# fgvieira/ngsF-HMM

Measured on AMD Instinct MI355X. Metric: site-ind updates/sec (EM iterations x individuals x sites / s), 1M sites x 1k ind, higher is better.
Workload: dtype f64

## Files before the change

### ngsf-hmm_amd/csrc/kernels_fast_estmaf.hip

```cpp
#include "fast_dev.hpp"

#include <mutex>

namespace capi {
void set_error(const char* fmt, ...);
}

namespace nghmm {

namespace {



__device__ double2 estmaf_term_logspace(const double* g, double freq, double F) {
  double h[3];
  h[0] = (1 - freq) * (1 - freq) + (1 - freq) * freq * F;
  h[1] = 2 * (1 - freq) * freq - 2 * (1 - freq) * freq * F;
  h[2] = freq * freq + (1 - freq) * freq * F;
  double pp[3];
  for (int k = 0; k < 3; ++k) {
    double l = log(h[k]);
    if (l == -__builtin_huge_val()) l = -kINF;
    h[k] = l;
  }
// ... 39 lines not shown
  {
    const uint64_t b = ngh_bits(v);
    const int lo = __builtin_amdgcn_update_dpp(0, (int)(uint32_t)b, 0x143, 0xc, 0xf, false);
    const int hi = __builtin_amdgcn_update_dpp(0, (int)(uint32_t)(b >> 32), 0x143, 0xc, 0xf, false);
    v += ngh_from_bits(((uint64_t)(uint32_t)hi << 32) | (uint32_t)lo);
  }
  return v;
}

__device__ __forceinline__ double wave_sum_uniform(double v) {
  v += dpp_move<0xB1>(v);
  v += dpp_move<0x4E>(v);
  v += dpp_move<0x141>(v);
  v += dpp_move<0x140>(v);
  return ((lane_value(v, 0) + lane_value(v, 16)) + lane_value(v, 32)) + lane_value(v, 48);
}

__device__ __forceinline__ double wave_sum_pair(double pn, double pd) {
  const uint64_t bn = ngh_bits(pn), bd = ngh_bits(pd);
  const auto lo = __builtin_amdgcn_permlane32_swap((unsigned)bn, (unsigned)bd, false, false);
  const auto hi = __builtin_amdgcn_permlane32_swap((unsigned)(bn >> 32), (unsigned)(bd >> 32),
                                                   false, false);
  double v = ngh_from_bits(((uint64_t)hi[0] << 32) | lo[0]) +
             ngh_from_bits(((uint64_t)hi[1] << 32) | lo[1]);
  v += dpp_move<0xB1>(v);
  v += dpp_move<0x4E>(v);
  v += dpp_move<0x141>(v);
  v += dpp_move<0x140>(v);
  {
    const uint64_t b = ngh_bits(v);
    const int l = __builtin_amdgcn_update_dpp(0, (int)(uint32_t)b, 0x142, 0xa, 0xf, false);
    const int h = __builtin_amdgcn_update_dpp(0, (int)(uint32_t)(b >> 32), 0x142, 0xa, 0xf, false);
    v += ngh_from_bits(((uint64_t)(uint32_t)h << 32) | (uint32_t)l);
  }
  return v;
}

constexpr int EN = 12;
constexpr int EST_SCALARS = 8;
constexpr int EST_FIELDS = EST_SCALARS + 2 * EN;
enum : uint8_t { EST_DONE = 0, EST_INTERP = 1, EST_EXACT = 2 };
constexpr int EST_K0 = 2;
constexpr int EST_MIN_GAIN = 24;
constexpr double EST_DMAX = 0.85;
constexpr double EST_BACK = 0.1;
constexpr double EST_MULT = 32.0;
constexpr double EST_FIT = 0.72;
constexpr int EST_KMAX = 32;
constexpr double EST_TOL = 1e-11;
constexpr double EST_GUARD = 1e-9;
__constant__ double kChebC[EN] = {0.9914448613738104, 0.9238795325112867, 0.7933533402912352, 0.6087614290087207, 0.38268343236508984, 0.1305261922200517, -0.1305261922200516, -0.3826834323650895, -0.6087614290087207, -0.793353340291235, -0.9238795325112867, -0.9914448613738104};
__constant__ double kChebW[EN] = {0.13052619222005157, -0.3826834323650898, 0.6087614290087207, -0.7933533402912352, 0.9238795325112867, -0.9914448613738104, 0.9914448613738104, -0.9238795325112868, 0.7933533402912352, -0.6087614290087209, 0.3826834323650899, -0.130526192220052};

constexpr int ESTMAF_MAXW = 16;

__device__ __forceinline__ bool in_tile_rows(uint64_t site, uint64_t tile_T, uint64_t row0,
                                             uint64_t row1) {
  if (tile_T == 0) return true;
  const uint64_t j = site / tile_T, t = site - j * tile_T;
  const uint64_t row = (j >> 6) * tile_T + t;
  return row >= row0 && row < row1;
}
__host__ __device__ constexpr int estmaf_full_slots(int NI, int BLOCK) {
  return BLOCK == 64 ? (NI == 16 ? 12 : NI == 12 ? 8 : NI == 8 ? 4 : NI == 4 ? 2 : NI == 2 ? 1 : 0)
                     : (NI == 16 ? 8 : 0);
}

template <int NI, int BLOCK, bool TILE>
__device__ __forceinline__ void estmaf_site(
    const GlView& gl, const double* __restrict__ marg_blocks, uint64_t S_own, uint64_t I_tot,
    uint64_t I_blk, double* __restrict__ freq_out, uint8_t* __restrict__ redo,
    uint8_t* __restrict__ status, double* __restrict__ state, uint64_t state_stride, int fresh,
    int n_exact, int allow_build, uint64_t site, const double* __restrict__ tile_col,
    uint32_t* __restrict__ cnt, double (&xch)[2][ESTMAF_MAXW][2],
    double2 (&nodebuf)[(BLOCK == 64 && NI >= 8) ? EN : 1][(BLOCK == 64 && NI >= 8) ? 65 : 1],
    double2 (&xnode)[(BLOCK == 64 && NI >= 8) ? 1 : EN][(BLOCK == 64 && NI >= 8) ? 1 : BLOCK / 64],
    double2* park = nullptr) {
  constexpr int W = BLOCK / 64;
  constexpr bool PARK = (W == 1 && NI >= 8);
  const int lane = threadIdx.x & 63;
  const int wv = threadIdx.x >> 6;
  const uint32_t tix = threadIdx.x;
  constexpr uint64_t stride = BLOCK;
  const uint64_t cell_s = site * I_tot;

  double tF_lane_out;
  double sA[NI], sb[NI], sC[NI], u0[NI], nC[NI], fc[NI];
  {
    constexpr int NB = NI < 8 ? NI : (NI % 8 ? NI / 2 : 8);
    static_assert(NI % NB == 0, "whole batches");
    const bool one_block = (I_blk == I_tot);
    const uint32_t ib = (uint32_t)I_blk;
    double tF_acc = 0;
#pragma unroll
    for (int k0 = 0; k0 < NI; k0 += NB) {
      double r0[NB], r1[NB], r2[NB], rF[NB];
      uint64_t ic[NB];
#pragma unroll
      for (int j = 0; j < NB; ++j) {
        const uint64_t i = (uint64_t)tix + stride * (k0 + j);
        ic[j] = (k0 + j < estmaf_full_slots(NI, BLOCK) || i < I_tot) ? i : I_tot - 1;
        gl_fetch(gl, cell_s + ic[j], r0[j], r1[j], r2[j]);
      }
      if constexpr (TILE) {
#pragma unroll
        for (int j = 0; j < NB; ++j)
          rF[j] = tile_col[k0 + j < estmaf_full_slots(NI, BLOCK)
// ... 47 lines not shown
    num = state[0 * state_stride + site];
    den = state[1 * state_stride + site];
    pnum = state[2 * state_stride + site];
    pden = state[3 * state_stride + site];
    iters = (int)state[4 * state_stride + site];
  }
  bool built = !allow_build;
  int n_before = n_exact;
  bool check = false, interp_ok = false;
  double mid = 0, half = 0, my_gn = 0, my_gd = 0, rprev = 0;
  auto lane_sums = [&](double r, double& pn, double& pd) {
    pn = 0;
    pd = 0;
    if constexpr (NI >= 4) {
#pragma unroll
      for (int k0 = 0; k0 + 4 <= NI; k0 += 4) {
        double sm[4];
#pragma unroll
        for (int j = 0; j < 4; ++j) sm[j] = fma(r, fma(r, sC[k0 + j], sb[k0 + j]), sA[k0 + j]);
        const double p01 = sm[0] * sm[1], p23 = sm[2] * sm[3];
        const double R = rcp_nr(p01 * p23);
        const double r01 = R * p23, r23 = R * p01;
        const double inv0 = r01 * sm[1], inv1 = r01 * sm[0];
        const double inv2 = r23 * sm[3], inv3 = r23 * sm[2];
        pn = fma(fma(nC[k0], r, u0[k0]), inv0, pn);
        pd = fma(fc[k0], inv0, pd);
        pn = fma(fma(nC[k0 + 1], r, u0[k0 + 1]), inv1, pn);
        pd = fma(fc[k0 + 1], inv1, pd);
        pn = fma(fma(nC[k0 + 2], r, u0[k0 + 2]), inv2, pn);
        pd = fma(fc[k0 + 2], inv2, pd);
        pn = fma(fma(nC[k0 + 3], r, u0[k0 + 3]), inv3, pn);
        pd = fma(fc[k0 + 3], inv3, pd);
      }
      if constexpr (NI % 4 == 2) {
        constexpr int k0 = NI - 2;
        const double s0 = fma(r, fma(r, sC[k0], sb[k0]), sA[k0]);
        const double s1 = fma(r, fma(r, sC[k0 + 1], sb[k0 + 1]), sA[k0 + 1]);
        const double R = rcp_nr(s0 * s1);
        const double inv0 = R * s1, inv1 = R * s0;
        pn = fma(fma(nC[k0], r, u0[k0]), inv0, pn);
        pd = fma(fc[k0], inv0, pd);
        pn = fma(fma(nC[k0 + 1], r, u0[k0 + 1]), inv1, pn);
        pd = fma(fc[k0 + 1], inv1, pd);
      }
    } else {
#pragma unroll
      for (int k = 0; k < NI; ++k) {
        const double inv = rcp_nr(fma(r, fma(r, sC[k], sb[k]), sA[k]));
        pn = fma(fma(nC[k], r, u0[k]), inv, pn);
        pd = fma(fc[k], inv, pd);
      }
    }
  };
  for (;;) {
    const double r = pnum * rcp_nr2(pden - pnum);
    double pn, pd;
    lane_sums(r, pn, pd);
    const double v = wave_sum_pair(pn, pd);
    double sn = lane_value(v, 31), sd = lane_value(v, 63);
    if constexpr (W > 1) {
      if (lane == 0) {
        xch[buf][wv][0] = sn;
        xch[buf][wv][1] = sd;
      }
      __syncthreads();
      sn = xch[buf][0][0];
      sd = xch[buf][0][1];
#pragma unroll
      for (int w = 1; w < W; ++w) {
        sn += xch[buf][w][0];
        sd += xch[buf][w][1];
      }
      buf ^= 1;
    }
    if (check) {
      const int nj = lane < EN ? lane : 0;
      const double t = (r - mid) / (r + mid) - half * kChebC[nj];
      const double q = (lane < EN) ? kChebW[nj] / t : 0.0;
      const double Sq = wave_sum_uniform(q);
      const double bn = wave_sum_uniform(q * my_gn) / Sq, bd = wave_sum_uniform(q * my_gd) / Sq;
      interp_ok = fabs(bn - sn) <= EST_TOL * fabs(sn) && fabs(bd - sd) <= EST_TOL * fabs(sd);
      check = false;
      if (!interp_ok && tix == 0) atomicAdd(cnt + EST_CNT_CHECK_FAILED, 1u);
    }
    num = fma(r, sn, num);
    den = fma(r, sd, den + tF_sum);
    const double lhs = fabs(fma(pnum, den, -(num * pden))), thr = kEPS * (den * pden);
    const bool again = (lhs > thr) && (iters++ < 100);
    rprev = r;
    pnum = num;
    pden = den;
    if (!again) break;
    if (interp_ok) {
      if (wv == 0) {
        if (lane < EN) {
          state[(EST_SCALARS + lane) * state_stride + site] = my_gn;
          state[(EST_SCALARS + EN + lane) * state_stride + site] = my_gd;
        }
        if (lane == 0) {
          state[0 * state_stride + site] = num;
          state[1 * state_stride + site] = den;
          state[2 * state_stride + site] = pnum;
          state[3 * state_stride + site] = pden;
          state[4 * state_stride + site] = (double)iters;
          state[5 * state_stride + site] = mid;
          state[6 * state_stride + site] = half;
          state[7 * state_stride + site] = tF_sum;
          status[site] = EST_INTERP;
        }
      }
      return;
    }
    if (!built && --n_before <= 0) {
      const double m_est = (double)iters * (sqrt(lhs / thr) - 1.0);
      const double rn = pnum * rcp_nr2(pden - pnum);
      const double step = fabs(rn - rprev);
      const double reach = (rn >= rprev) ? EST_DMAX * rn : EST_DMAX / (1 + EST_DMAX) * rn;
      const bool fits = (double)iters * step <= EST_FIT * reach;
      if (!fits && iters < EST_KMAX && m_est >= EST_MIN_GAIN) {
        n_before = 1;
      } else {
        built = true;
      }
      if (built && m_est >= EST_MIN_GAIN && 100 - iters >= EST_MIN_GAIN) {
        const double g = fmin(EST_DMAX, fmax(EST_MULT * step / rn, 1e-3));
        double lo, hi;
        if (rn >= rprev) {
          lo = rn * (1 - EST_BACK * g);
          hi = rn * (1 + g);
        } else {
          lo = rn / (1 + g);
          hi = rn * (1 + EST_BACK * g);
        }
        mid = sqrt(lo * hi);
        half = (hi - mid) / (hi + mid);
        if (half > 0 && lo > 0 && hi < 1e300) {
          if constexpr (PARK) {
            const double tnl = half * kChebC[lane < EN ? lane : 0];
            const double r_nodes = mid * (1 + tnl) * rcp_nr2(1 - tnl);
#pragma unroll 1
            for (int nd = 0; nd < EN; ++nd) {
              double pn, pd;
              lane_sums(lane_value(r_nodes, nd), pn, pd);
              nodebuf[nd][lane] = double2{pn, pd};
            }
            __syncthreads();
            const int j = lane & 15, q4 = lane >> 4;
            double an = 0, ad = 0;
            if (j < EN) {
#pragma unroll
              for (int l = 0; l < 16; ++l) {
                const double2 t2 = nodebuf[j][q4 * 16 + l];
                an += t2.x;
                ad += t2.y;
              }
            }
            an += __shfl_xor(an, 16);
            ad += __shfl_xor(ad, 16);
            an += __shfl_xor(an, 32);
            ad += __shfl_xor(ad, 32);
            my_gn = an;
            my_gd = ad;
            check = true;
          } else {
            const double tnl = half * kChebC[lane < EN ? lane : 0];
            const double r_nodes = mid * (1 + tnl) * rcp_nr2(1 - tnl);
            double an = 0, ad = 0;
            if constexpr (W > 1) {
#pragma unroll 1
              for (int nd = 0; nd < EN; ++nd) {
                double pn, pd;
                lane_sums(lane_value(r_nodes, nd), pn, pd);
                park[nd * BLOCK + (int)tix] = double2{pn, pd};
              }
              __syncthreads();
              for (int nd = wv; nd < EN; nd += W) {
                double sn = 0, sd = 0;
#pragma unroll
                for (int w = 0; w < W; ++w) {
                  const double2 t2 = park[nd * BLOCK + w * 64 + lane];
                  sn += t2.x;
                  sd += t2.y;
                }
                const double v = wave_sum_pair(sn, sd);
                const double tn = lane_value(v, 31), td = lane_value(v, 63);
                if (lane == 0) xnode[nd][0] = double2{tn, td};
              }
              __syncthreads();
              if (lane < EN) {
                an = xnode[lane][0].x;
                ad = xnode[lane][0].y;
              }
              __syncthreads();
            } else {
#pragma unroll 1
              for (int nd = 0; nd < EN; ++nd) {
                double pn, pd;
                lane_sums(lane_value(r_nodes, nd), pn, pd);
                const double v = wave_sum_pair(pn, pd);
                const double sn = lane_value(v, 31), sd = lane_value(v, 63);
                if (lane == nd) {
                  an = sn;
                  ad = sd;
                }
              }
            }
            my_gn = an;
            my_gd = ad;
            check = true;
          }
        }
      }
    }
  }
  if (tix == 0) {
    const double freq = num / den;
    const bool ok = freq >= 0 && freq < 1;
    freq_out[site] = freq;
    redo[site] = ok ? 0 : 1;
    status[site] = EST_DONE;
  }
}

__device__ __forceinline__ const double* estmaf_tile_col(const double* marg_blocks, uint64_t site,
                                                         uint64_t tile_T, uint64_t I_tot) {
  const uint64_t j = site / tile_T, t = site - j * tile_T;
  return marg_blocks + post_lane_off((j >> 6) * tile_T + t, j & 63, I_tot);
}

#define ESTMAF_SHARED(NI, BLOCK)                                                              \
  constexpr bool PARK_ = ((BLOCK) == 64 && (NI) >= 8);                                         \
  __shared__ double xch[2][ESTMAF_MAXW][2];                       \
  __shared__ double2 nodebuf[PARK_ ? EN : 1][PARK_ ? 65 : 1];                                  \
  __shared__ double2 xnode[PARK_ ? 1 : EN][PARK_ ? 1 : (BLOCK) / 64]

template <int NI, int BLOCK, bool TILE>
__global__ void __launch_bounds__(BLOCK) __attribute__((amdgpu_waves_per_eu(2)))
k_fast_estmaf(const GlView gl, const double* __restrict__ marg_blocks,
              uint64_t S_own, uint64_t I_tot, uint64_t I_blk, uint64_t tile_T,
              double* __restrict__ freq_out, uint8_t* __restrict__ redo,
              uint8_t* __restrict__ status, double* __restrict__ state, uint64_t state_stride,
              int n_exact, int allow_build, uint64_t blk0, uint32_t* __restrict__ cnt) {
  ESTMAF_SHARED(NI, BLOCK);
  uint64_t site;
  const double* tile_col = nullptr;
  if constexpr (TILE) {
    const uint64_t b = blockIdx.x + blk0, x = b & 7, k = b >> 3;
    const uint64_t q = ((k >> 3) << 6) + (x << 3) + (k & 7);
    const uint64_t tile_row = q >> 6, l = q & 63;
    const uint64_t c = tile_row / tile_T, t = tile_row - c * tile_T;
    site = (c * 64 + l) * tile_T + t;
    if (site >= S_own) return;
    tile_col = marg_blocks + post_lane_off(tile_row, l, I_tot);
  } else {
    site = blockIdx.x;
  }
  extern __shared__ double2 park_mem[];
  estmaf_site<NI, BLOCK, TILE>(gl, marg_blocks, S_own, I_tot, I_blk, freq_out, redo, status, state,
                               state_stride, 1, n_exact, allow_build, site, tile_col, cnt, xch, nodebuf,
                               xnode, park_mem);
}

template <int NI, int BLOCK, bool TILE>
__global__ void __launch_bounds__(BLOCK) __attribute__((amdgpu_waves_per_eu(2)))
k_fast_estmaf_resume(const GlView gl, const double* __restrict__ marg_blocks,
                     uint64_t S_own, uint64_t I_tot, uint64_t I_blk, uint64_t tile_T,
                     double* __restrict__ freq_out, uint8_t* __restrict__ redo,
                     uint8_t* __restrict__ status, double* __restrict__ state,
                     uint64_t state_stride, int n_exact, int allow_build, uint64_t row0,
                     uint64_t row1, uint32_t* __restrict__ cnt, int cnt_slot) {
  ESTMAF_SHARED(NI, BLOCK);
  extern __shared__ double2 park_mem[];
  const int lane = threadIdx.x & 63;
  for (uint64_t base = (uint64_t)blockIdx.x * 64; base < S_own; base += (uint64_t)gridDim.x * 64) {
    const uint64_t s = base + lane;
    const bool need = s < S_own && in_tile_rows(s, TILE ? tile_T : 0, row0, row1) &&
                      status[s] == EST_EXACT;
    uint64_t mask = __ballot(need);
    if (mask && threadIdx.x == 0) atomicAdd(cnt + cnt_slot, (uint32_t)__popcll(mask));
    if constexpr (BLOCK > 64) __syncthreads();
    while (mask) {
      const uint64_t site = base + (uint64_t)__builtin_ctzll(mask);
      mask &= mask - 1;
      const double* tile_col = TILE ? estmaf_tile_col(marg_blocks, site, tile_T, I_tot) : nullptr;
      estmaf_site<NI, BLOCK, TILE>(gl, marg_blocks, S_own, I_tot, I_blk, freq_out, redo, status,
                                   state, state_stride, 0, n_exact, allow_build, site, tile_col, cnt,
                                   xch, nodebuf, xnode, park_mem);
      if constexpr (BLOCK > 64) __syncthreads();
    }
  }
}

__device__ __forceinline__ double row_sum(double v) {
  v = __dadd_rn(v, dpp_move<0xB1>(v));
  v = __dadd_rn(v, dpp_move<0x4E>(v));
  v = __dadd_rn(v, dpp_move<0x141>(v));
  v = __dadd_rn(v, dpp_move<0x140>(v));
  return v;
}

template <int NI, bool TILE>
__device__ __forceinline__ void estmaf_rows_sites(
    const GlView& gl, const double* __restrict__ marg_blocks, uint64_t S_own, uint64_t I_tot,
    uint64_t I_blk, double* __restrict__ freq_out, uint8_t* __restrict__ redo,
    uint8_t* __restrict__ status, double* __restrict__ state, uint64_t state_stride, int fresh,
    int n_exact, int allow_build, uint64_t site, const double* __restrict__ tile_col, bool done,
    uint32_t* __restrict__ cnt) {
  static_assert(EN <= 16, "a row's lanes hold the interval's node sums");
  const int lane = threadIdx.x, j = lane & 15;
  const uint64_t cell_s = site * I_tot;

  double sA[NI], sb[NI], sC[NI], u0[NI], nC[NI], fc[NI];
  double tF_acc = 0;
  {
    const bool one_block = (I_blk == I_tot);
    const uint32_t ib = (uint32_t)I_blk;
    double r0[NI], r1[NI], r2[NI], rF[NI];
    uint64_t ic[NI];
#pragma unroll
    for (int k = 0; k < NI; ++k) {
      const uint64_t i = (uint64_t)j + 16 * k;
      ic[k] = i < I_tot ? i : I_tot - 1;
      gl_fetch(gl, cell_s + ic[k], r0[k], r1[k], r2[k]);
    }
#pragma unroll
    for (int k = 0; k < NI; ++k) {
      if constexpr (TILE) {
        rF[k] = tile_col[post_ind_off(ic[k])];
      } else if (one_block) {
        rF[k] = marg_blocks[site * I_blk + ic[k]];
      } else {
        const uint32_t q = (uint32_t)ic[k] / ib;
        rF[k] = marg_blocks[((uint64_t)q * S_own + site) * I_blk + ((uint32_t)ic[k] - q * ib)];
      }
    }
#pragma unroll
    for (int k = 0; k < NI; ++k) {
      const bool valid = (uint64_t)j + 16 * k < I_tot;
      const double p0 = valid ? r0[k] : 1.0, p1 = valid ? r1[k] : 0.0;
      const double p2 = valid ? r2[k] : 0.0, F = valid ? rF[k] : 0.0;
      const double cc = p1 * fma(-2.0, F, 2.0);
      const double n2 = (2 - F) * p2;
      sA[k] = p0;
      sb[k] = fma(F, p0 + p2, cc);
      sC[k] = p2;
      u0[k] = fma(n2, F, cc);
      nC[k] = n2;
      fc[k] = F * cc;
      tF_acc += valid ? 2 - F : 0.0;
    }
  }
  const double tF_sum = row_sum(tF_acc);

  int iters = 0;
  double num = 0, den = 0;
  double pnum = 0.01, pden = 1.0;
  if (!fresh && !done) {
    num = state[0 * state_stride + site];
    den = state[1 * state_stride + site];
    pnum = state[2 * state_stride + site];
    pden = state[3 * state_stride + site];
    iters = (int)state[4 * state_stride + site];
  }
  bool built = !allow_build;
  int n_before = n_exact;
  bool check = false;
  double mid = 1, half = 0.5, my_gn = 0, my_gd = 0, rprev = 0;
  auto lane_sums = [&](double r, double& pn, double& pd) {
    pn = 0;
    pd = 0;
    if constexpr (NI >= 4) {
#pragma unroll
      for (int k0 = 0; k0 < NI; k0 += 4) {
        double sm[4];
#pragma unroll
        for (int k = 0; k < 4; ++k) sm[k] = fma(r, fma(r, sC[k0 + k], sb[k0 + k]), sA[k0 + k]);
        const double p01 = sm[0] * sm[1], p23 = sm[2] * sm[3];
        const double R = rcp_nr(p01 * p23);
        const double r01 = R * p23, r23 = R * p01;
        const double inv0 = r01 * sm[1], inv1 = r01 * sm[0];
        const double inv2 = r23 * sm[3], inv3 = r23 * sm[2];
        pn = fma(fma(nC[k0], r, u0[k0]), inv0, pn);
        pd = fma(fc[k0], inv0, pd);
        pn = fma(fma(nC[k0 + 1], r, u0[k0 + 1]), inv1, pn);
        pd = fma(fc[k0 + 1], inv1, pd);
        pn = fma(fma(nC[k0 + 2], r, u0[k0 + 2]), inv2, pn);
        pd = fma(fc[k0 + 2], inv2, pd);
        pn = fma(fma(nC[k0 + 3], r, u0[k0 + 3]), inv3, pn);
        pd = fma(fc[k0 + 3], inv3, pd);
      }
    } else {
#pragma unroll
      for (int k = 0; k < NI; ++k) {
        const double inv = rcp_nr(fma(r, fma(r, sC[k], sb[k]), sA[k]));
        pn = fma(fma(nC[k], r, u0[k]), inv, pn);
        pd = fma(fc[k], inv, pd);
      }
    }
  };
  for (;;) {
    const double r = pnum * rcp_nr2(pden - pnum);
    double pn, pd;
    lane_sums(r, pn, pd);
    const double sn = row_sum(pn), sd = row_sum(pd);
    bool interp_ok = false;
    if (__builtin_amdgcn_ballot_w64(check && !done) != 0) {
      const int nj = j < EN ? j : 0;
      const double t = (r - mid) / (r + mid) - half * kChebC[nj];
      const double q = (j < EN) ? kChebW[nj] / t : 0.0;
      const double Sq = row_sum(q);
      const double bn = row_sum(q * my_gn) / Sq, bd = row_sum(q * my_gd) / Sq;
      if (check && !done) {
        interp_ok = fabs(bn - sn) <= EST_TOL * fabs(sn) && fabs(bd - sd) <= EST_TOL * fabs(sd);
        if (!interp_ok && j == 0) atomicAdd(cnt + EST_CNT_CHECK_FAILED, 1u);
      }
      check = false;
    }
    bool want_build = false;
    if (!done) {
      num = fma(r, sn, num);
      den = fma(r, sd, den + tF_sum);
      const double lhs = fabs(fma(pnum, den, -(num * pden))), thr = kEPS * (den * pden);
      const bool again = (lhs > thr) && (iters++ < 100);
      rprev = r;
      pnum = num;
      pden = den;
      if (!again) {
        if (j == 0) {
          const double freq = num / den;
          const bool ok = freq >= 0 && freq < 1;
          freq_out[site] = freq;
          redo[site] = ok ? 0 : 1;
          status[site] = EST_DONE;
        }
        done = true;
      } else if (interp_ok) {
        if (j < EN) {
          state[(EST_SCALARS + j) * state_stride + site] = my_gn;
          state[(EST_SCALARS + EN + j) * state_stride + site] = my_gd;
        }
        if (j == 0) {
          state[0 * state_stride + site] = num;
          state[1 * state_stride + site] = den;
          state[2 * state_stride + site] = pnum;
          state[3 * state_stride + site] = pden;
          state[4 * state_stride + site] = (double)iters;
          state[5 * state_stride + site] = mid;
          state[6 * state_stride + site] = half;
          state[7 * state_stride + site] = tF_sum;
          status[site] = EST_INTERP;
        }
        done = true;
      } else if (!built && --n_before <= 0) {
        const double m_est = (double)iters * (sqrt(lhs / thr) - 1.0);
        const double rn = pnum * rcp_nr2(pden - pnum);
        const double step = fabs(rn - rprev);
        const double reach = (rn >= rprev) ? EST_DMAX * rn : EST_DMAX / (1 + EST_DMAX) * rn;
        const bool fits = (double)iters * step <= EST_FIT * reach;
        if (!fits && iters < EST_KMAX && m_est >= EST_MIN_GAIN) {
          n_before = 1;
        } else {
          built = true;
        }
        if (built && m_est >= EST_MIN_GAIN && 100 - iters >= EST_MIN_GAIN) {
          const double g = fmin(EST_DMAX, fmax(EST_MULT * step / rn, 1e-3));
          double lo, hi;
          if (rn >= rprev) {
            lo = rn * (1 - EST_BACK * g);
            hi = rn * (1 + g);
          } else {
            lo = rn / (1 + g);
            hi = rn * (1 + EST_BACK * g);
          }
          const double a = sqrt(lo * hi), h = (hi - a) / (hi + a);
          if (h > 0 && lo > 0 && hi < 1e300) {
            mid = a;
            half = h;
            want_build = true;
          }
        }
      }
    }
    if (__builtin_amdgcn_ballot_w64(want_build) != 0) {
#pragma unroll 1
      for (int nd = 0; nd < EN; ++nd) {
        const double tn = half * kChebC[nd];
        double qn, qd;
        lane_sums(mid * (1 + tn) * rcp_nr2(1 - tn), qn, qd);
        const double gn = row_sum(qn), gd = row_sum(qd);
        if (want_build && j == nd) {
          my_gn = gn;
          my_gd = gd;
        }
      }
      if (want_build) check = true;
    }
    if (__builtin_amdgcn_ballot_w64(!done) == 0) break;
  }
}

template <int NI, bool TILE>
__global__ void __launch_bounds__(64)
k_fast_estmaf_rows(const GlView gl, const double* __restrict__ marg_blocks, uint64_t S_own,
                   uint64_t I_tot, uint64_t I_blk, uint64_t tile_T, double* __restrict__ freq_out,
                   uint8_t* __restrict__ redo, uint8_t* __restrict__ status,
                   double* __restrict__ state, uint64_t state_stride, int n_exact,
                   int allow_build, uint32_t* __restrict__ cnt) {
  const int lane = threadIdx.x, row = lane >> 4;
  uint64_t site;
  const double* tile_col = nullptr;
  if constexpr (TILE) {
    const uint64_t b = blockIdx.x, x = b & 7, k = b >> 3;
    const uint64_t q = ((k >> 1) << 6) + (x << 3) + ((k & 1) << 2) + row;
    const uint64_t tile_row = q >> 6, l = q & 63;
    const uint64_t c = tile_row / tile_T, t = tile_row - c * tile_T;
    site = (c * 64 + l) * tile_T + t;
    tile_col = marg_blocks + post_lane_off(tile_row, l, I_tot);
  } else {
    site = (uint64_t)blockIdx.x * 4 + row;
  }
  bool done = site >= S_own;
  if (done) {
    site = 0;
    if constexpr (TILE) tile_col = marg_blocks;
  }
  if (__builtin_amdgcn_ballot_w64(!done) == 0) return;
  estmaf_rows_sites<NI, TILE>(gl, marg_blocks, S_own, I_tot, I_blk, freq_out, redo, status, state,
                              state_stride, 1, n_exact, allow_build, site, tile_col, done, cnt);
}

template <int NI, bool TILE>
__global__ void __launch_bounds__(64)
k_fast_estmaf_rows_resume(const GlView gl, const double* __restrict__ marg_blocks, uint64_t S_own,
                          uint64_t I_tot, uint64_t I_blk, uint64_t tile_T,
                          double* __restrict__ freq_out, uint8_t* __restrict__ redo,
                          uint8_t* __restrict__ status, double* __restrict__ state,
                          uint64_t state_stride, int n_exact, int allow_build,
                          uint32_t* __restrict__ cnt, int cnt_slot) {
  const int lane = threadIdx.x, row = lane >> 4;
  for (uint64_t base = (uint64_t)blockIdx.x * 64; base < S_own; base += (uint64_t)gridDim.x * 64) {
    const uint64_t s = base + lane;
    uint64_t mask = __ballot(s < S_own && status[s] == EST_EXACT);
    if (mask && lane == 0) atomicAdd(cnt + cnt_slot, (uint32_t)__popcll(mask));
    while (mask) {
      uint64_t site = 0;
      bool done = true;
#pragma unroll
      for (int r = 0; r < 4; ++r) {
        if (mask) {
          const uint64_t cand = base + (uint64_t)__builtin_ctzll(mask);
          mask &= mask - 1;
          if (r == row) {
            site = cand;
            done = false;
          }
        }
      }
      const double* tile_col =
          TILE ? (done ? marg_blocks : estmaf_tile_col(marg_blocks, site, tile_T, I_tot)) : nullptr;
      estmaf_rows_sites<NI, TILE>(gl, marg_blocks, S_own, I_tot, I_blk, freq_out, redo, status,
                                  state, state_stride, 0, n_exact, allow_build, site, tile_col, done,
                                  cnt);
    }
  }
}

__global__ void __launch_bounds__(256)
k_fast_estmaf_interp(uint64_t S_own, double* __restrict__ freq_out, uint8_t* __restrict__ redo,
                     uint8_t* __restrict__ status, double* __restrict__ state,
                     uint64_t state_stride, uint64_t tile_T, uint64_t row0, uint64_t row1) {
  const uint64_t site = (uint64_t)blockIdx.x * blockDim.x + threadIdx.x;
  if (site >= S_own || !in_tile_rows(site, tile_T, row0, row1) || status[site] != EST_INTERP)
    return;
  double num = state[0 * state_stride + site], den = state[1 * state_stride + site];
  double pnum = state[2 * state_stride + site], pden = state[3 * state_stride + site];
  int iters = (int)state[4 * state_stride + site];
  const double mid = state[5 * state_stride + site], half = state[6 * state_stride + site];
  const double tF_sum = state[7 * state_stride + site];
  double gn[EN], gd[EN];
#pragma unroll
  for (int j = 0; j < EN; ++j) {
    gn[j] = state[(EST_SCALARS + j) * state_stride + site];
    gd[j] = state[(EST_SCALARS + EN + j) * state_stride + site];
  }
  double cn[EN], cd[EN];
#pragma unroll
  for (int k = 0; k < EN; ++k) cn[k] = cd[k] = 0;
#pragma unroll
  for (int j = 0; j < EN; ++j) {
    const double x = kChebC[j], fn = gn[j] * (2.0 / EN), fd = gd[j] * (2.0 / EN);
    double t0 = 1.0, t1 = x;
    cn[0] += fn;
    cd[0] += fd;
#pragma unroll
    for (int k = 1; k < EN; ++k) {
      cn[k] = fma(fn, t1, cn[k]);
      cd[k] = fma(fd, t1, cd[k]);
      const double t2 = fma(2 * x, t1, -t0);
      t0 = t1;
      t1 = t2;
    }
  }
  const double inv_half = 1.0 / half;
  uint8_t st = EST_EXACT;
  for (;;) {
    const double r = pnum * rcp_nr2(pden - pnum);
    const double tt = (r - mid) * rcp_nr2(r + mid);
    if (!(fabs(tt) <= half)) break;
    const double x2 = 2 * (tt * inv_half);
    double bn1 = 0, bn2 = 0, bd1 = 0, bd2 = 0;
#pragma unroll
    for (int k = EN - 1; k >= 1; --k) {
      const double bn0 = fma(x2, bn1, cn[k] - bn2), bd0 = fma(x2, bd1, cd[k] - bd2);
      bn2 = bn1;
      bn1 = bn0;
      bd2 = bd1;
      bd1 = bd0;
    }
    const double sn = fma(0.5 * x2, bn1, 0.5 * cn[0] - bn2);
    const double sd = fma(0.5 * x2, bd1, 0.5 * cd[0] - bd2);
    const double num2 = fma(r, sn, num), den2 = fma(r, sd, den + tF_sum);
    const double lhs = fabs(fma(pnum, den2, -(num2 * pden))), thr = kEPS * (den2 * pden);
    if (!(fabs(lhs - thr) >= EST_GUARD * thr)) break;
    num = num2;
    den = den2;
    const bool again = (lhs > thr) && (iters++ < 100);
    pnum = num;
    pden = den;
    if (!again) {
      st = EST_DONE;
      break;
    }
  }
  if (st == EST_DONE) {
    const double freq = num / den;
    const bool ok = freq >= 0 && freq < 1;
    freq_out[site] = freq;
    redo[site] = ok ? 0 : 1;
  } else {
    state[0 * state_stride + site] = num;
    state[1 * state_stride + site] = den;
    state[2 * state_stride + site] = pnum;
    state[3 * state_stride + site] = pden;
    state[4 * state_stride + site] = (double)iters;
  }
  status[site] = st;
}

constexpr int ESTC_A0 = 0, ESTC_B0 = 1, ESTC_M0 = 2, ESTC_M1 = 3, ESTC_M2 = 4;

template <bool TILE>
__global__ void __launch_bounds__(64)
k_fast_estmaf_called_sums(const GlView gl, const double* __restrict__ marg_blocks, uint64_t S_own,
                          uint64_t I_tot, uint64_t I_blk, uint64_t tile_T,
                          uint8_t* __restrict__ redo, double* __restrict__ state,
                          uint64_t state_stride, uint64_t blk0) {
  const int lane = threadIdx.x;
  uint64_t site;
  const double* tile_col = nullptr;
  if constexpr (TILE) {
    const uint64_t b = blockIdx.x + blk0, x = b & 7, k = b >> 3;
    const uint64_t q = ((k >> 3) << 6) + (x << 3) + (k & 7);
    const uint64_t tile_row = q >> 6, l = q & 63;
    const uint64_t c = tile_row / tile_T, t = tile_row - c * tile_T;
    site = (c * 64 + l) * tile_T + t;
    if (site >= S_own) return;
    tile_col = marg_blocks + post_lane_off(tile_row, l, I_tot);
  } else {
    site = blockIdx.x;
  }
  const uint64_t cell_s = gl.cell0 + site * I_tot;
  const bool one_block = (I_blk == I_tot);
  double n1 = 0, s2 = 0, s02 = 0, m0 = 0, m1 = 0, m2 = 0;
  bool bad = false;
  auto posterior = [&](uint64_t i) -> double {
    if constexpr (TILE) return tile_col[post_ind_off(i)];
    if (one_block) return marg_blocks[site * I_blk + i];
    const uint64_t q = i / I_blk;
    return marg_blocks[(q * S_own + site) * I_blk + (i - q * I_blk)];
  };
  auto take = [&](uint32_t code, double F) {
    const double tF = 2 - F;
    const bool g1 = code == 1, g2 = code == 2, g3 = code == 3;
    n1 += g1 ? 1.0 : 0.0;
    bad |= g1 && !(F < 1);
    s2 += g2 ? tF : 0.0;
    s02 += (code == 0 || g2) ? tF : 0.0;
    m0 += g3 ? 1 - F : 0.0;
    m1 += g3 ? tF : 0.0;
    m2 += g3 ? F * tF : 0.0;
  };
  uint64_t i = lane;
  for (; i + 192 < I_tot; i += 256) {
    double F[4];
    uint32_t cd[4];
#pragma unroll
    for (int j = 0; j < 4; ++j) {
// ... 95 lines not shown
    num += wave_sum(pn);
    den += wave_sum(pd);
    freq = num / den;
    again = (fabs(prev - freq) > kEPS) && (iters++ < 100);
  } while (again);
  if (lane == 0) freq_out[site] = freq;
}

__global__ void __launch_bounds__(256)
k_fast_estmaf_stream(const GlView gl, const double* __restrict__ marg_blocks,
                     uint64_t S_own, uint64_t I_tot, uint64_t I_blk, uint64_t tile_T,
                     double* __restrict__ freq_out, const uint8_t* __restrict__ redo,
                     uint64_t row0, uint64_t row1, uint32_t* __restrict__ cnt) {
  const int lane = threadIdx.x & 63;
  const uint64_t wave = (uint64_t)blockIdx.x * (blockDim.x >> 6) + (threadIdx.x >> 6);
  const uint64_t n_waves = (uint64_t)gridDim.x * (blockDim.x >> 6);
  if (!redo) {
    for (uint64_t site = wave; site < S_own; site += n_waves)
      if (in_tile_rows(site, tile_T, row0, row1))
        estmaf_stream_site(gl, marg_blocks, S_own, I_tot, I_blk, tile_T, freq_out, site, lane);
    return;
  }
  for (uint64_t base = wave * 64; base < S_own; base += n_waves * 64) {
    const uint64_t s = base + lane;
    const bool need = s < S_own && in_tile_rows(s, tile_T, row0, row1) && redo[s];
    uint64_t mask = __ballot(need);
    if (mask && lane == 0) atomicAdd(cnt + EST_CNT_LOGSPACE, (uint32_t)__popcll(mask));
    while (mask) {
      const int b = __builtin_ctzll(mask);
      mask &= mask - 1;
      estmaf_stream_site(gl, marg_blocks, S_own, I_tot, I_blk, tile_T, freq_out, base + b, lane);
    }
  }
}

}


bool fast_estmaf_called(const FastState& fs, const GlView& gl) {
  return !gl.dense && gl.codes && fs.called_table && !fs.sw.estmaf_no_called;
}

bool fast_estmaf_in_place(const FastState& fs, uint64_t I_tot) {
  return I_tot <= 8192 || (fs.packed && fs.called_table && !fs.sw.estmaf_no_called);
}

bool fast_estmaf_splittable(const FastState& fs, uint64_t I_tot, bool tile_major) {
  if (tile_major && fs.packed && fs.called_table && !fs.sw.estmaf_no_called) return true;
  return tile_major && I_tot > 128 && I_tot <= 8192;
}

bool fast_estmaf_reserve(FastState& fs, uint64_t S_own) {
  if (!fs.est_counts) {
    if (hipMalloc((void**)&fs.est_counts, EST_COUNTS * sizeof(uint32_t)) != hipSuccess) return false;
    if (hipMemset(fs.est_counts, 0, EST_COUNTS * sizeof(uint32_t)) != hipSuccess) return false;
    if (hipDeviceSynchronize() != hipSuccess) return false;
  }
  if (S_own <= fs.redo_cap) return true;
  if (fs.redo) (void)hipFree(fs.redo);
  if (fs.est_status) (void)hipFree(fs.est_status);
  if (fs.est_state) (void)hipFree(fs.est_state);
  fs.redo = fs.est_status = nullptr;
  fs.est_state = nullptr;
  fs.redo_cap = 0;
  if (hipMalloc((void**)&fs.redo, S_own) != hipSuccess) return false;
  if (hipMalloc((void**)&fs.est_status, S_own) != hipSuccess) return false;
  if (hipMalloc((void**)&fs.est_state, S_own * EST_FIELDS * sizeof(double)) != hipSuccess) return false;
  fs.redo_cap = S_own;
  return true;
}

static bool estmaf_dyn_lds(const void* kernel, size_t bytes) {
  if (bytes <= 65536) return true;
  static std::vector<std::pair<const void*, int>> told;
  static std::mutex mu;
  int dev = 0;
  (void)hipGetDevice(&dev);
  std::lock_guard<std::mutex> lock(mu);
  const std::pair<const void*, int> key{kernel, dev};
  if (std::find(told.begin(), told.end(), key) != told.end()) return true;
  const hipError_t e =
      hipFuncSetAttribute(kernel, hipFuncAttributeMaxDynamicSharedMemorySize, (int)bytes);
  if (e != hipSuccess) {
    (void)hipGetLastError();
    capi::set_error("est_maf: the kernel needs %zu bytes of dynamic LDS per workgroup and the "
                    "device refuses them (hipFuncSetAttribute: %s)", bytes, hipGetErrorString(e));
    return false;
  }
  told.push_back(key);
  return true;
}

bool fast_estmaf(FastState& fs, hipStream_t st, const GlView& d_gl_sites,
                 const double* d_marg_blocks, uint64_t S_own, uint64_t I_tot, uint64_t I_blk,
                 double* d_freq_out, bool tile_major, uint32_t part, uint32_t n_parts) {
  if (S_own == 0) return true;
  if (n_parts == 0 || part >= n_parts) return false;
  if (n_parts > 1 && !fast_estmaf_splittable(fs, I_tot, tile_major)) return false;
  const uint64_t n_rows = (uint64_t)fs.C * fs.T;
  const uint64_t row0 = n_parts > 1 ? n_rows * part / n_parts : 0;
  const uint64_t row1 = n_parts > 1 ? n_rows * (part + 1) / n_parts : n_rows;
  const uint64_t blk0 = row0 * 64, nblk = (row1 - row0) * 64;
  if (nblk == 0) return true;
  if (tile_major && !((I_tot <= 8192 || fast_estmaf_called(fs, d_gl_sites)) && I_blk == I_tot &&
                      S_own == fs.S))
    return false;
  const uint64_t tile_T = tile_major ? fs.T : 0;
  const bool stream_all = I_tot > 8192 && !tile_major;
  const uint64_t stream_wgs = stream_all ? (S_own + 3) / 4 : (S_own + 255) / 256;
  const dim3 grid((unsigned)(stream_wgs < 65536 ? stream_wgs : 65536)), block(256);
  if (!fast_estmaf_reserve(fs, S_own)) return false;
  if (fast_estmaf_called(fs, d_gl_sites)) {
    if (tile_major)
      hipLaunchKernelGGL((k_fast_estmaf_called_sums<true>), dim3((unsigned)nblk), dim3(64), 0, st,
                         d_gl_sites, d_marg_blocks, S_own, I_tot, I_blk, tile_T, fs.redo, fs.est_state,
                         fs.redo_cap, blk0);
    else
      hipLaunchKernelGGL((k_fast_estmaf_called_sums<false>), dim3((unsigned)S_own), dim3(64), 0, st,
                         d_gl_sites, d_marg_blocks, S_own, I_tot, I_blk, tile_T, fs.redo, fs.est_state,
                         fs.redo_cap, (uint64_t)0);
    hipLaunchKernelGGL(k_fast_estmaf_called_passes, dim3((unsigned)((S_own + 255) / 256)), dim3(256), 0,
                       st, S_own, d_freq_out, fs.redo, fs.est_status, fs.est_state, fs.redo_cap, tile_T,
                       row0, row1);
    hipLaunchKernelGGL(k_fast_estmaf_stream, grid, block, 0, st, d_gl_sites, d_marg_blocks, S_own,
                       I_tot, I_blk, tile_T, d_freq_out, fs.redo, row0, row1, fs.est_counts);
    return hipGetLastError() == hipSuccess;
  }
  bool interp = true;
  interp = fs.sw.estmaf_interp != 0;
  const uint64_t scan_wgs_all = (S_own + 63) / 64;
  const unsigned scan_wgs = (unsigned)(scan_wgs_all < 16384 ? scan_wgs_all : 16384);
#define ESTMAF_DYN(B) ((B) > 64 ? (size_t)EN * (B) * sizeof(double2) : (size_t)0)
#define ESTMAF_TELL(K, B) estmaf_dyn_lds(reinterpret_cast<const void*>(K), ESTMAF_DYN(B))
#define LAUNCH_NI(N, B)                                                                         \
  do {                                                                                          \
    if (fresh) {                                                                                \
      if (!ESTMAF_TELL((k_fast_estmaf<N, B, false>), B)) return false;                          \
      hipLaunchKernelGGL((k_fast_estmaf<N, B, false>), dim3((unsigned)S_own), dim3(B),          \
                         ESTMAF_DYN(B), st, d_gl_sites, d_marg_blocks, S_own, I_tot, I_blk,     \
                         (uint64_t)0, d_freq_out, fs.redo, fs.est_status, fs.est_state,         \
                         fs.redo_cap, n_exact, allow_build, (uint64_t)0, fs.est_counts);        \
    } else {                                                                                    \
      if (!ESTMAF_TELL((k_fast_estmaf_resume<N, B, false>), B)) return false;                   \
      hipLaunchKernelGGL((k_fast_estmaf_resume<N, B, false>), dim3(scan_wgs), dim3(B),          \
                         ESTMAF_DYN(B), st, d_gl_sites, d_marg_blocks, S_own, I_tot, I_blk,     \
                         (uint64_t)0, d_freq_out, fs.redo, fs.est_status, fs.est_state,         \
                         fs.redo_cap, n_exact, allow_build, row0, row1, fs.est_counts,          \
                         cnt_slot);                                                             \
    }                                                                                           \
  } while (0)
#define LAUNCH_TILE(N, B)                                                                       \
  do {                                                                                          \
    if (fresh) {                                                                                \
      if (!ESTMAF_TELL((k_fast_estmaf<N, B, true>), B)) return false;                           \
      hipLaunchKernelGGL((k_fast_estmaf<N, B, true>), dim3((unsigned)nblk), dim3(B),            \
                         ESTMAF_DYN(B), st, d_gl_sites, d_marg_blocks, S_own, I_tot, I_blk,     \
                         tile_T, d_freq_out, fs.redo, fs.est_status, fs.est_state, fs.redo_cap, \
                         n_exact, allow_build, blk0, fs.est_counts);                            \
    } else {                                                                                    \
      if (!ESTMAF_TELL((k_fast_estmaf_resume<N, B, true>), B)) return false;                    \
      hipLaunchKernelGGL((k_fast_estmaf_resume<N, B, true>), dim3(scan_wgs), dim3(B),           \
                         ESTMAF_DYN(B), st, d_gl_sites, d_marg_blocks, S_own, I_tot, I_blk,     \
                         tile_T, d_freq_out, fs.redo, fs.est_status, fs.est_state, fs.redo_cap, \
                         n_exact, allow_build, row0, row1, fs.est_counts, cnt_slot);            \
    }                                                                                           \
  } while (0)
#define LAUNCH_ROWS(N, TL)                                                                      \
  do {                                                                                          \
    if (fresh)                                                                                  \
      hipLaunchKernelGGL((k_fast_estmaf_rows<N, TL>),                                            \
                         dim3((unsigned)((TL) ? fs.Spad / 4 : (S_own + 3) / 4)), dim3(64), 0,   \
                         st, d_gl_sites, d_marg_blocks, S_own, I_tot, I_blk, tile_T, d_freq_out, \
                         fs.redo, fs.est_status, fs.est_state, fs.redo_cap, n_exact,            \
                         allow_build, fs.est_counts);                                           \
    else                                                                                        \
      hipLaunchKernelGGL((k_fast_estmaf_rows_resume<N, TL>), dim3(scan_wgs), dim3(64), 0, st,    \
                         d_gl_sites, d_marg_blocks, S_own, I_tot, I_blk, tile_T, d_freq_out,    \
                         fs.redo, fs.est_status, fs.est_state, fs.redo_cap, n_exact,            \
                         allow_build, fs.est_counts, cnt_slot);                                 \
  } while (0)
  const bool rows = I_tot <= 128 && !fs.sw.estmaf_no_rows;
  auto launch = [&](int fresh, int n_exact, int allow_build, int cnt_slot = 0) -> bool {
    if (rows) {
      if (tile_major) {
        if (I_tot <= 16) LAUNCH_ROWS(1, true);
        else if (I_tot <= 32) LAUNCH_ROWS(2, true);
        else if (I_tot <= 64) LAUNCH_ROWS(4, true);
        else LAUNCH_ROWS(8, true);
      } else {
        if (I_tot <= 16) LAUNCH_ROWS(1, false);
        else if (I_tot <= 32) LAUNCH_ROWS(2, false);
        else if (I_tot <= 64) LAUNCH_ROWS(4, false);
        else LAUNCH_ROWS(8, false);
      }
      return true;
    }
    if (tile_major) {
      if (I_tot <= 64) LAUNCH_TILE(1, 64);
      else if (I_tot <= 128) LAUNCH_TILE(2, 64);
      else if (I_tot <= 256) LAUNCH_TILE(4, 64);
      else if (I_tot <= 512) LAUNCH_TILE(8, 64);
      else if (I_tot <= 768) LAUNCH_TILE(12, 64);
      else if (I_tot <= 1024) LAUNCH_TILE(16, 64);
      else if (I_tot <= 1536) LAUNCH_TILE(12, 128);
      else if (I_tot <= 2048) LAUNCH_TILE(16, 128);
      else if (I_tot <= 3072) LAUNCH_TILE(12, 256);
      else if (I_tot <= 4096) LAUNCH_TILE(16, 256);
      else if (I_tot <= 5120) LAUNCH_TILE(10, 512);
      else if (I_tot <= 6144) LAUNCH_TILE(12, 512);
      else if (I_tot <= 7168) LAUNCH_TILE(14, 512);
      else LAUNCH_TILE(16, 512);
    } else if (I_tot <= 64) LAUNCH_NI(1, 64);
    else if (I_tot <= 128) LAUNCH_NI(2, 64);
    else if (I_tot <= 256) LAUNCH_NI(4, 64);
    else if (I_tot <= 512) LAUNCH_NI(8, 64);
    else if (I_tot <= 768) LAUNCH_NI(12, 64);
    else if (I_tot <= 1024) LAUNCH_NI(16, 64);
    else if (I_tot <= 1536) LAUNCH_NI(12, 128);
    else if (I_tot <= 2048) LAUNCH_NI(16, 128);
    else if (I_tot <= 3072) LAUNCH_NI(12, 256);
    else if (I_tot <= 4096) LAUNCH_NI(16, 256);
    else if (I_tot <= 5120) LAUNCH_NI(10, 512);
    else if (I_tot <= 6144) LAUNCH_NI(12, 512);
    else if (I_tot <= 7168) LAUNCH_NI(14, 512);
    else LAUNCH_NI(16, 512);
    return true;
  };
  const uint8_t* redo = fs.redo;
  if (I_tot > 8192 && !tile_major) {
    redo = nullptr;
  } else if (!interp) {
    if (!launch(1, 0, 0)) return false;
  } else {
    const dim3 igrid((unsigned)((S_own + 255) / 256));
    if (!launch(1, EST_K0, 1)) return false;
    hipLaunchKernelGGL(k_fast_estmaf_interp, igrid, dim3(256), 0, st, S_own, d_freq_out, fs.redo,
                       fs.est_status, fs.est_state, fs.redo_cap, tile_T, row0, row1);
    for (int again = 0; again < 2; ++again) {
      if (!launch(0, 1, 1, again ? EST_CNT_RESUMED_AGAIN : EST_CNT_RESUMED)) return false;
      hipLaunchKernelGGL(k_fast_estmaf_interp, igrid, dim3(256), 0, st, S_own, d_freq_out, fs.redo,
                         fs.est_status, fs.est_state, fs.redo_cap, tile_T, row0, row1);
    }
    if (!launch(0, 0, 0, EST_CNT_EXACT_TAIL)) return false;
  }
  hipLaunchKernelGGL(k_fast_estmaf_stream, grid, block, 0, st, d_gl_sites, d_marg_blocks, S_own,
                     I_tot, I_blk, tile_T, d_freq_out, redo, row0, row1, fs.est_counts);
#undef LAUNCH_NI
#undef ESTMAF_DYN
#undef ESTMAF_TELL
#undef LAUNCH_TILE
#undef LAUNCH_ROWS
  return hipGetLastError() == hipSuccess;
}

}
```

Before: 42.48 billion.

## Certify Chebyshev interpolant by coefficient decay and skip empty resume passes

```diff
diff --git a/ngsf-hmm_amd/csrc/kernels_fast_estmaf.hip b/ngsf-hmm_amd/csrc/kernels_fast_estmaf.hip
--- a/ngsf-hmm_amd/csrc/kernels_fast_estmaf.hip
+++ b/ngsf-hmm_amd/csrc/kernels_fast_estmaf.hip
@@ -115,7 +115,42 @@
 __constant__ double kChebC[EN] = {0.9914448613738104, 0.9238795325112867, 0.7933533402912352, 0.6087614290087207, 0.38268343236508984, 0.1305261922200517, -0.1305261922200516, -0.3826834323650895, -0.6087614290087207, -0.793353340291235, -0.9238795325112867, -0.9914448613738104};
 __constant__ double kChebW[EN] = {0.13052619222005157, -0.3826834323650898, 0.6087614290087207, -0.7933533402912352, 0.9238795325112867, -0.9914448613738104, 0.9914448613738104, -0.9238795325112868, 0.7933533402912352, -0.6087614290087209, 0.3826834323650899, -0.130526192220052};
 
+constexpr double EST_CERT = 2e-9;
+__constant__ double kCertT[64] = {
+    0.16666666666666666, 0.16666666666666666, 0.16666666666666666, 0.16666666666666666, 0.16666666666666666, 0.16666666666666666, 0.16666666666666666, 0.16666666666666666, 0.16666666666666666, 0.16666666666666666, 0.16666666666666666, 0.16666666666666666, 0.0, 0.0, 0.0, 0.0,
+    0.0637805720608483, -0.15397992208521447, 0.15397992208521447, -0.0637805720608483, -0.06378057206084842, 0.15397992208521444, -0.15397992208521438, 0.06378057206084825, 0.06378057206084847, -0.1539799220852146, 0.15397992208521447, -0.06378057206084765, 0.0, 0.0, 0.0, 0.0,
+    0.04313650751708679, -0.11785113019775798, 0.1609876377148447, -0.1609876377148447, 0.11785113019775796, -0.04313650751708693, -0.04313650751708685, 0.1178511301977579, -0.16098763771484467, 0.16098763771484476, -0.11785113019775811, 0.04313650751708713, 0.0, 0.0, 0.0, 0.0,
+    0.02175436537000862, -0.06378057206084825, 0.10146023816812005, -0.13222555671520586, 0.15397992208521444, -0.1652408102289684, 0.16524081022896836, -0.15397992208521427, 0.13222555671520608, -0.10146023816812022, 0.06378057206084818, -0.021754365370008216, 0.0, 0.0, 0.0, 0.0};
+
+__device__ __forceinline__ double row_sum(double v) {
+  v = __dadd_rn(v, dpp_move<0xB1>(v));
+  v = __dadd_rn(v, dpp_move<0x4E>(v));
+  v = __dadd_rn(v, dpp_move<0x141>(v));
+  v = __dadd_rn(v, dpp_move<0x140>(v));
+  return v;
+}
+
+__device__ __forceinline__ bool cheb_certify(double gn, double gd) {
+  const double t = kCertT[threadIdx.x & 63];
+  const double vn = row_sum(gn * t), vd = row_sum(gd * t);
+  const double tail_n = fmax(fmax(fabs(lane_value(vn, 16)), fabs(lane_value(vn, 32))), fabs(lane_value(vn, 48)));
+  const double tail_d = fmax(fmax(fabs(lane_value(vd, 16)), fabs(lane_value(vd, 32))), fabs(lane_value(vd, 48)));
+  return tail_n <= EST_CERT * fabs(lane_value(vn, 0)) && tail_d <= EST_CERT * fabs(lane_value(vd, 0));
+}
+__device__ __forceinline__ bool cheb_certify_row(double gn, double gd) {
+  const int j = threadIdx.x & 15;
+  const double c0n = row_sum(gn * kCertT[j]), c0d = row_sum(gd * kCertT[j]);
+  double tail_n = 0, tail_d = 0;
+#pragma unroll
+  for (int q = 1; q < 4; ++q) {
+    tail_n = fmax(tail_n, fabs(row_sum(gn * kCertT[16 * q + j])));
+    tail_d = fmax(tail_d, fabs(row_sum(gd * kCertT[16 * q + j])));
+  }
+  return tail_n <= EST_CERT * fabs(c0n) && tail_d <= EST_CERT * fabs(c0d);
+}
+
 constexpr int ESTMAF_MAXW = 16;
+constexpr int EST_PEND_STAGES = 4, EST_PEND_PARTS = 16;
 
 __device__ __forceinline__ bool in_tile_rows(uint64_t site, uint64_t tile_T, uint64_t row0,
                                              uint64_t row1) {
@@ -269,6 +304,25 @@
       }
     }
   };
+  auto hand_over = [&]() {
+    if (wv == 0) {
+      if (lane < EN) {
+        state[(EST_SCALARS + lane) * state_stride + site] = my_gn;
+        state[(EST_SCALARS + EN + lane) * state_stride + site] = my_gd;
+      }
+      if (lane == 0) {
+        state[0 * state_stride + site] = num;
+        state[1 * state_stride + site] = den;
+        state[2 * state_stride + site] = pnum;
+        state[3 * state_stride + site] = pden;
+        state[4 * state_stride + site] = (double)iters;
+        state[5 * state_stride + site] = mid;
+        state[6 * state_stride + site] = half;
+        state[7 * state_stride + site] = tF_sum;
+        status[site] = EST_INTERP;
+      }
+    }
+  };
   for (;;) {
     const double r = pnum * rcp_nr2(pden - pnum);
     double pn, pd;
@@ -298,7 +352,6 @@
       const double bn = wave_sum_uniform(q * my_gn) / Sq, bd = wave_sum_uniform(q * my_gd) / Sq;
       interp_ok = fabs(bn - sn) <= EST_TOL * fabs(sn) && fabs(bd - sd) <= EST_TOL * fabs(sd);
       check = false;
-      if (!interp_ok && tix == 0) atomicAdd(cnt + EST_CNT_CHECK_FAILED, 1u);
     }
     num = fma(r, sn, num);
     den = fma(r, sd, den + tF_sum);
@@ -309,23 +362,7 @@
     pden = den;
     if (!again) break;
     if (interp_ok) {
-      if (wv == 0) {
-        if (lane < EN) {
-          state[(EST_SCALARS + lane) * state_stride + site] = my_gn;
-          state[(EST_SCALARS + EN + lane) * state_stride + site] = my_gd;
-        }
-        if (lane == 0) {
-          state[0 * state_stride + site] = num;
-          state[1 * state_stride + site] = den;
-          state[2 * state_stride + site] = pnum;
-          state[3 * state_stride + site] = pden;
-          state[4 * state_stride + site] = (double)iters;
-          state[5 * state_stride + site] = mid;
-          state[6 * state_stride + site] = half;
-          state[7 * state_stride + site] = tF_sum;
-          status[site] = EST_INTERP;
-        }
-      }
+      hand_over();
       return;
     }
     if (!built && --n_before <= 0) {
@@ -378,7 +415,6 @@
             ad += __shfl_xor(ad, 32);
             my_gn = an;
             my_gd = ad;
-            check = true;
           } else {
             const double tnl = half * kChebC[lane < EN ? lane : 0];
             const double r_nodes = mid * (1 + tnl) * rcp_nr2(1 - tnl);
@@ -404,9 +440,9 @@
                 if (lane == 0) xnode[nd][0] = double2{tn, td};
               }
               __syncthreads();
-              if (lane < EN) {
-                an = xnode[lane][0].x;
-                ad = xnode[lane][0].y;
+              if ((lane & 15) < EN) {
+                an = xnode[lane & 15][0].x;
+                ad = xnode[lane & 15][0].y;
               }
               __syncthreads();
             } else {
@@ -416,7 +452,7 @@
                 lane_sums(lane_value(r_nodes, nd), pn, pd);
                 const double v = wave_sum_pair(pn, pd);
                 const double sn = lane_value(v, 31), sd = lane_value(v, 63);
-                if (lane == nd) {
+                if ((lane & 15) == nd) {
                   an = sn;
                   ad = sd;
                 }
@@ -424,8 +460,13 @@
             }
             my_gn = an;
             my_gd = ad;
-            check = true;
           }
+          if (cheb_certify(my_gn, my_gd)) {
+            hand_over();
+            return;
+          }
+          if (tix == 0) atomicAdd(cnt + EST_CNT_CHECK_FAILED, 1u);
+          check = true;
         }
       }
     }
@@ -485,7 +526,9 @@
                      double* __restrict__ freq_out, uint8_t* __restrict__ redo,
                      uint8_t* __restrict__ status, double* __restrict__ state,
                      uint64_t state_stride, int n_exact, int allow_build, uint64_t row0,
-                     uint64_t row1, uint32_t* __restrict__ cnt, int cnt_slot) {
+                     uint64_t row1, uint32_t* __restrict__ cnt, int cnt_slot,
+                     const uint32_t* __restrict__ pend) {
+  if (pend && *pend == 0) return;
   ESTMAF_SHARED(NI, BLOCK);
   extern __shared__ double2 park_mem[];
   const int lane = threadIdx.x & 63;
@@ -508,13 +551,6 @@
   }
 }
 
-__device__ __forceinline__ double row_sum(double v) {
-  v = __dadd_rn(v, dpp_move<0xB1>(v));
-  v = __dadd_rn(v, dpp_move<0x4E>(v));
-  v = __dadd_rn(v, dpp_move<0x141>(v));
-  v = __dadd_rn(v, dpp_move<0x140>(v));
-  return v;
-}
 
 template <int NI, bool TILE>
 __device__ __forceinline__ void estmaf_rows_sites(
@@ -615,6 +651,23 @@
       }
     }
   };
+  auto hand_over = [&]() {
+    if (j < EN) {
+      state[(EST_SCALARS + j) * state_stride + site] = my_gn;
+      state[(EST_SCALARS + EN + j) * state_stride + site] = my_gd;
+    }
+    if (j == 0) {
+      state[0 * state_stride + site] = num;
+      state[1 * state_stride + site] = den;
+      state[2 * state_stride + site] = pnum;
+      state[3 * state_stride + site] = pden;
+      state[4 * state_stride + site] = (double)iters;
+      state[5 * state_stride + site] = mid;
+      state[6 * state_stride + site] = half;
+      state[7 * state_stride + site] = tF_sum;
+      status[site] = EST_INTERP;
+    }
+  };
   for (;;) {
     const double r = pnum * rcp_nr2(pden - pnum);
     double pn, pd;
@@ -627,10 +680,8 @@
       const double q = (j < EN) ? kChebW[nj] / t : 0.0;
       const double Sq = row_sum(q);
       const double bn = row_sum(q * my_gn) / Sq, bd = row_sum(q * my_gd) / Sq;
-      if (check && !done) {
+      if (check && !done)
         interp_ok = fabs(bn - sn) <= EST_TOL * fabs(sn) && fabs(bd - sd) <= EST_TOL * fabs(sd);
-        if (!interp_ok && j == 0) atomicAdd(cnt + EST_CNT_CHECK_FAILED, 1u);
-      }
       check = false;
     }
     bool want_build = false;
@@ -652,21 +703,7 @@
         }
         done = true;
       } else if (interp_ok) {
-        if (j < EN) {
-          state[(EST_SCALARS + j) * state_stride + site] = my_gn;
-          state[(EST_SCALARS + EN + j) * state_stride + site] = my_gd;
-        }
-        if (j == 0) {
-          state[0 * state_stride + site] = num;
-          state[1 * state_stride + site] = den;
-          state[2 * state_stride + site] = pnum;
-          state[3 * state_stride + site] = pden;
-          state[4 * state_stride + site] = (double)iters;
-          state[5 * state_stride + site] = mid;
-          state[6 * state_stride + site] = half;
-          state[7 * state_stride + site] = tF_sum;
-          status[site] = EST_INTERP;
-        }
+        hand_over();
         done = true;
       } else if (!built && --n_before <= 0) {
         const double m_est = (double)iters * (sqrt(lhs / thr) - 1.0);
@@ -710,7 +747,16 @@
           my_gd = gd;
         }
       }
-      if (want_build) check = true;
+      const bool cert = cheb_certify_row(my_gn, my_gd);
+      if (want_build) {
+        if (cert) {
+          hand_over();
+          done = true;
+        } else {
+          if (j == 0) atomicAdd(cnt + EST_CNT_CHECK_FAILED, 1u);
+          check = true;
+        }
+      }
     }
     if (__builtin_amdgcn_ballot_w64(!done) == 0) break;
   }
@@ -753,7 +799,9 @@
                           double* __restrict__ freq_out, uint8_t* __restrict__ redo,
                           uint8_t* __restrict__ status, double* __restrict__ state,
                           uint64_t state_stride, int n_exact, int allow_build,
-                          uint32_t* __restrict__ cnt, int cnt_slot) {
+                          uint32_t* __restrict__ cnt, int cnt_slot,
+                          const uint32_t* __restrict__ pend) {
+  if (pend && *pend == 0) return;
   const int lane = threadIdx.x, row = lane >> 4;
   for (uint64_t base = (uint64_t)blockIdx.x * 64; base < S_own; base += (uint64_t)gridDim.x * 64) {
     const uint64_t s = base + lane;
@@ -785,7 +833,9 @@
 __global__ void __launch_bounds__(256)
 k_fast_estmaf_interp(uint64_t S_own, double* __restrict__ freq_out, uint8_t* __restrict__ redo,
                      uint8_t* __restrict__ status, double* __restrict__ state,
-                     uint64_t state_stride, uint64_t tile_T, uint64_t row0, uint64_t row1) {
+                     uint64_t state_stride, uint64_t tile_T, uint64_t row0, uint64_t row1,
+                     const uint32_t* __restrict__ pend_in, uint32_t* __restrict__ pend_out) {
+  if (pend_in && *pend_in == 0) return;
   const uint64_t site = (uint64_t)blockIdx.x * blockDim.x + threadIdx.x;
   if (site >= S_own || !in_tile_rows(site, tile_T, row0, row1) || status[site] != EST_INTERP)
     return;
@@ -860,6 +910,10 @@
     state[2 * state_stride + site] = pnum;
     state[3 * state_stride + site] = pden;
     state[4 * state_stride + site] = (double)iters;
+    if (pend_out) {
+      const uint64_t m = __ballot(1);
+      if ((threadIdx.x & 63) == (unsigned)__builtin_ctzll(m)) atomicAdd(pend_out, (uint32_t)__popcll(m));
+    }
   }
   status[site] = st;
 }
@@ -1061,8 +1115,9 @@
 
 bool fast_estmaf_reserve(FastState& fs, uint64_t S_own) {
   if (!fs.est_counts) {
-    if (hipMalloc((void**)&fs.est_counts, EST_COUNTS * sizeof(uint32_t)) != hipSuccess) return false;
-    if (hipMemset(fs.est_counts, 0, EST_COUNTS * sizeof(uint32_t)) != hipSuccess) return false;
+    constexpr size_t n_words = EST_COUNTS + (size_t)EST_PEND_PARTS * EST_PEND_STAGES;
+    if (hipMalloc((void**)&fs.est_counts, n_words * sizeof(uint32_t)) != hipSuccess) return false;
+    if (hipMemset(fs.est_counts, 0, n_words * sizeof(uint32_t)) != hipSuccess) return false;
     if (hipDeviceSynchronize() != hipSuccess) return false;
   }
   if (S_own <= fs.redo_cap) return true;
@@ -1155,7 +1210,7 @@
                          ESTMAF_DYN(B), st, d_gl_sites, d_marg_blocks, S_own, I_tot, I_blk,     \
                          (uint64_t)0, d_freq_out, fs.redo, fs.est_status, fs.est_state,         \
                          fs.redo_cap, n_exact, allow_build, row0, row1, fs.est_counts,          \
-                         cnt_slot);                                                             \
+                         cnt_slot, pend);                                                          \
     }                                                                                           \
   } while (0)
 #define LAUNCH_TILE(N, B)                                                                       \
@@ -1171,7 +1226,7 @@
       hipLaunchKernelGGL((k_fast_estmaf_resume<N, B, true>), dim3(scan_wgs), dim3(B),           \
                          ESTMAF_DYN(B), st, d_gl_sites, d_marg_blocks, S_own, I_tot, I_blk,     \
                          tile_T, d_freq_out, fs.redo, fs.est_status, fs.est_state, fs.redo_cap, \
-                         n_exact, allow_build, row0, row1, fs.est_counts, cnt_slot);            \
+                         n_exact, allow_build, row0, row1, fs.est_counts, cnt_slot, pend);      \
     }                                                                                           \
   } while (0)
 #define LAUNCH_ROWS(N, TL)                                                                      \
@@ -1186,10 +1241,11 @@
       hipLaunchKernelGGL((k_fast_estmaf_rows_resume<N, TL>), dim3(scan_wgs), dim3(64), 0, st,    \
                          d_gl_sites, d_marg_blocks, S_own, I_tot, I_blk, tile_T, d_freq_out,    \
                          fs.redo, fs.est_status, fs.est_state, fs.redo_cap, n_exact,            \
-                         allow_build, fs.est_counts, cnt_slot);                                 \
+                         allow_build, fs.est_counts, cnt_slot, pend);                           \
   } while (0)
   const bool rows = I_tot <= 128 && !fs.sw.estmaf_no_rows;
-  auto launch = [&](int fresh, int n_exact, int allow_build, int cnt_slot = 0) -> bool {
+  auto launch = [&](int fresh, int n_exact, int allow_build, int cnt_slot = 0,
+                    const uint32_t* pend = nullptr) -> bool {
     if (rows) {
       if (tile_major) {
         if (I_tot <= 16) LAUNCH_ROWS(1, true);
@@ -1242,15 +1298,20 @@
     if (!launch(1, 0, 0)) return false;
   } else {
     const dim3 igrid((unsigned)((S_own + 255) / 256));
+    uint32_t* pend = part < (uint32_t)EST_PEND_PARTS ? fs.est_counts + EST_COUNTS + part * EST_PEND_STAGES : nullptr;
+    if (pend && hipMemsetAsync(pend, 0, EST_PEND_STAGES * sizeof(uint32_t), st) != hipSuccess) return false;
     if (!launch(1, EST_K0, 1)) return false;
     hipLaunchKernelGGL(k_fast_estmaf_interp, igrid, dim3(256), 0, st, S_own, d_freq_out, fs.redo,
-                       fs.est_status, fs.est_state, fs.redo_cap, tile_T, row0, row1);
+                       fs.est_status, fs.est_state, fs.redo_cap, tile_T, row0, row1,
+                       (const uint32_t*)nullptr, pend);
     for (int again = 0; again < 2; ++again) {
-      if (!launch(0, 1, 1, again ? EST_CNT_RESUMED_AGAIN : EST_CNT_RESUMED)) return false;
+      const uint32_t* before = pend ? pend + again : nullptr;
+      if (!launch(0, 1, 1, again ? EST_CNT_RESUMED_AGAIN : EST_CNT_RESUMED, before)) return false;
       hipLaunchKernelGGL(k_fast_estmaf_interp, igrid, dim3(256), 0, st, S_own, d_freq_out, fs.redo,
-                         fs.est_status, fs.est_state, fs.redo_cap, tile_T, row0, row1);
-    }
-    if (!launch(0, 0, 0, EST_CNT_EXACT_TAIL)) return false;
+                         fs.est_status, fs.est_state, fs.redo_cap, tile_T, row0, row1, before,
+                         pend ? pend + again + 1 : nullptr);
+    }
+    if (!launch(0, 0, 0, EST_CNT_EXACT_TAIL, pend ? pend + 2 : nullptr)) return false;
   }
   hipLaunchKernelGGL(k_fast_estmaf_stream, grid, block, 0, st, d_gl_sites, d_marg_blocks, S_own,
                      I_tot, I_blk, tile_T, d_freq_out, redo, row0, row1, fs.est_counts);
```

Result: no change. 43.06 billion, median of 6 (+1.4%).
